# TianyiFranklinWang/MIRROR

Hardware: AMD Instinct MI355X
Metric: SSL samples/sec (slide+RNA pairs) (higher is better)
Workload: dtype bf16; 1 GPU; BASELINE c2: B=16/GPU x [4096 patch tokens x 1024-d] + [2048 genes], D=512, RNA depth 6 / 8 heads, train mode, local-batch InfoNCE; precision_policy=bf16, per_gpu_batch=16, global_batch=16, parallelism=dp1, grad_bucket_dtype=f32, step_launch=hip_graph

## Files before the change

### mirror_amd/csrc/resconv_mfma.hip

```cpp
#include <cstdlib>
#include "gemm_kernel.h"

namespace {

constexpr int RM_P = 72;
constexpr int RM_T = 128;
constexpr int RM_HALO = 16;
constexpr int RM_TAPS = 33;
constexpr int RM_DH = 64;
constexpr int RM_SP = 68;

typedef __attribute__((address_space(3))) s16x4 lds_s16x4;
typedef short s16x8 __attribute__((ext_vector_type(8)));
#define MFMA(a, b, c) __builtin_amdgcn_mfma_f32_32x32x16_bf16((a), (b), (c), 0, 0, 0)

__device__ __forceinline__ bf16x8 rm_frag_tr(const bf16_t* img, int col0, int kb, int lane) {
    const int g16 = lane >> 4, i = lane & 15, q = i >> 2, p = i & 3;
    const bf16_t* a0 = img + (kb + 4 * (g16 >> 1) + q) * RM_P + col0 + 16 * (g16 & 1) + 4 * p;
    s16x4 lo = __builtin_amdgcn_ds_read_tr16_b64_v4i16((lds_s16x4*)a0);
    s16x4 hi = __builtin_amdgcn_ds_read_tr16_b64_v4i16((lds_s16x4*)(a0 + 8 * RM_P));
    s16x8 v = __builtin_shufflevector(lo, hi, 0, 1, 2, 3, 4, 5, 6, 7);
    return __builtin_bit_cast(bf16x8, v);
}

__global__ __launch_bounds__(256) void resconv_mfma_kernel(const bf16_t* __restrict__ v, long ldv, long v_bs, const float* __restrict__ w,
                                                           bf16_t* out, long ldo, long o_bs, int n_p, int transpose, int accumulate) {
    static_assert(64 * RM_SP * 4 <= (RM_T + 2 * RM_HALO) * RM_P * 2, "half of the f32 output image must fit the v tile");
    __shared__ __attribute__((aligned(16))) bf16_t img[(RM_T + 2 * RM_HALO) * RM_P];
    const int tid = threadIdx.x, lane = tid & 63, wave = tid >> 6, hl = lane >> 5, r = lane & 31;
    const int t0 = blockIdx.x * RM_T, h = blockIdx.y, b = blockIdx.z;
    const bf16_t* vb = v + (long)b * v_bs + h * RM_DH;
#pragma unroll
    for (int i = 0; i < (RM_T + 2 * RM_HALO) * 8 / 256; i++) {
        const int cid = tid + i * 256, q = cid >> 3, c = cid & 7;
        const int t = t0 - RM_HALO + q;
        u32x4 val = {0u, 0u, 0u, 0u};
        if (t >= 0 && t < n_p) val = *reinterpret_cast<const u32x4*>(vb + (long)t * ldv + c * 8);
        *reinterpret_cast<u32x4*>(img + q * RM_P + c * 8) = val;
    }
    bf16_t* ob = out + (long)b * o_bs + h * RM_DH;
    u32x4 old[2][64 * 8 / 256];
    if (accumulate == 2) {
#pragma unroll
        for (int half = 0; half < 2; half++)
#pragma unroll
            for (int i = 0; i < 64 * 8 / 256; i++) {
                const int cid = tid + i * 256, q = cid >> 3, c = cid & 7;
                const int t = t0 + 64 * half + q;
                old[half][i] = (u32x4){0u, 0u, 0u, 0u};
                if (t < n_p) old[half][i] = *reinterpret_cast<const u32x4*>(ob + (long)t * ldo + 8 * c);
            }
    }
    const float* wh = w + h * RM_TAPS;
    bf16x8 wf[4];
#pragma unroll
    for (int ks = 0; ks < 4; ks++)
#pragma unroll
        for (int e = 0; e < 8; e++) {
            const int k = 16 * ks + (e < 4 ? 4 * hl + e : 8 + 4 * hl + (e - 4));
            const int j = k - r;
            const float x = (j >= 0 && j < RM_TAPS) ? wh[transpose ? RM_TAPS - 1 - j : j] : 0.f;
            wf[ks][e] = (__bf16)x;
        }
    __syncthreads();
    f32x16 acc[2];
#pragma unroll
    for (int nb = 0; nb < 2; nb++) {
#pragma unroll
        for (int e = 0; e < 16; e++) acc[nb][e] = 0.f;
#pragma unroll
        for (int ks = 0; ks < 4; ks++) acc[nb] = MFMA(rm_frag_tr(img, 32 * nb, 32 * wave + 16 * ks, lane), wf[ks], acc[nb]);
    }
    float* stage = reinterpret_cast<float*>(img);
    __syncthreads();
#pragma unroll
    for (int half = 0; half < 2; half++) {
        if ((wave >> 1) == half) {
            float* srow = stage + (32 * (wave & 1) + r) * RM_SP + 4 * hl;
#pragma unroll
            for (int nb = 0; nb < 2; nb++)
#pragma unroll
                for (int g = 0; g < 4; g++) {
                    f4_t x = {acc[nb][4 * g], acc[nb][4 * g + 1], acc[nb][4 * g + 2], acc[nb][4 * g + 3]};
                    *reinterpret_cast<f4_t*>(srow + 32 * nb + 8 * g) = x;
                }
        }
        __syncthreads();
#pragma unroll
        for (int i = 0; i < 64 * 8 / 256; i++) {
            const int cid = tid + i * 256, q = cid >> 3, c = cid & 7;
            const int t = t0 + 64 * half + q;
            if (t >= n_p) continue;
            const float* sp = stage + q * RM_SP + 8 * c;
            f4_t lo = *reinterpret_cast<const f4_t*>(sp), hi = *reinterpret_cast<const f4_t*>(sp + 4);
            bf16_t* p = ob + (long)t * ldo + 8 * c;
            if (accumulate) {
                const u32x4 od = accumulate == 2 ? old[half][i] : *reinterpret_cast<const u32x4*>(p);
                lo[0] += __uint_as_float(od[0] << 16); lo[1] += __uint_as_float(od[0] & 0xffff0000u);
                lo[2] += __uint_as_float(od[1] << 16); lo[3] += __uint_as_float(od[1] & 0xffff0000u);
                hi[0] += __uint_as_float(od[2] << 16); hi[1] += __uint_as_float(od[2] & 0xffff0000u);
                hi[2] += __uint_as_float(od[3] << 16); hi[3] += __uint_as_float(od[3] & 0xffff0000u);
            }
            u32x4 o;
            o[0] = pack_bf2(lo[0], lo[1]);
            o[1] = pack_bf2(lo[2], lo[3]);
            o[2] = pack_bf2(hi[0], hi[1]);
            o[3] = pack_bf2(hi[2], hi[3]);
            __builtin_nontemporal_store(o, reinterpret_cast<u32x4*>(p));
        }
        if (half == 0) __syncthreads();
    }
}

__global__ __launch_bounds__(256) void resconv_wgrad_mfma_kernel(const bf16_t* __restrict__ v, long ldv, long v_bs,
                                                                 const bf16_t* __restrict__ dout, long ldo, long o_bs,
                                                                 float* __restrict__ dw, int n_p) {
    __shared__ float gsum[64];
    __shared__ float s_S[4 * 32 * 65];
    const int tid = threadIdx.x, lane = tid & 63, wave = tid >> 6, hl = lane >> 5, r = lane & 31;
    const int h = blockIdx.y, b = blockIdx.z;
    if (tid < 64) gsum[tid] = 0.f;
    const bf16_t* vb = v + (long)b * v_bs + h * RM_DH + 8 * hl;
    const bf16_t* gb = dout + (long)b * o_bs + h * RM_DH + 8 * hl;
    f32x16 acc[2];
#pragma unroll
    for (int kb = 0; kb < 2; kb++)
#pragma unroll
        for (int e = 0; e < 16; e++) acc[kb][e] = 0.f;
    const int nblk = (n_p + 31) / 32;
    auto fetch = [&](int tb, bf16x8 (&af)[4], bf16x8 (&bf)[2][4]) {
        const int t = 32 * tb + r;
        const bool tok = t < n_p;
#pragma unroll
        for (int ks = 0; ks < 4; ks++) {
            u32x4 a = {0u, 0u, 0u, 0u};
            if (tok) a = *reinterpret_cast<const u32x4*>(gb + (long)t * ldo + 16 * ks);
            af[ks] = __builtin_bit_cast(bf16x8, a);
        }
#pragma unroll
        for (int kb = 0; kb < 2; kb++) {
            const int q = 32 * tb - RM_HALO + 32 * kb + r;
            const bool qok = q >= 0 && q < n_p;
#pragma unroll
            for (int ks = 0; ks < 4; ks++) {
                u32x4 x = {0u, 0u, 0u, 0u};
                if (qok) x = *reinterpret_cast<const u32x4*>(vb + (long)q * ldv + 16 * ks);
                bf[kb][ks] = __builtin_bit_cast(bf16x8, x);
            }
        }
    };
    auto mac = [&](const bf16x8 (&af)[4], const bf16x8 (&bf)[2][4]) {
#pragma unroll
        for (int kb = 0; kb < 2; kb++)
#pragma unroll
            for (int ks = 0; ks < 4; ks++) acc[kb] = MFMA(af[ks], bf[kb][ks], acc[kb]);
    };
    const int stride = 4 * gridDim.x;
    int tb = blockIdx.x * 4 + wave;
    bf16x8 a0[4], b0[2][4], a1[4], b1[2][4];
    if (tb < nblk) fetch(tb, a0, b0);
    while (tb < nblk) {
        if (tb + stride < nblk) fetch(tb + stride, a1, b1);
        mac(a0, b0);
        tb += stride;
        if (tb >= nblk) break;
        if (tb + stride < nblk) fetch(tb + stride, a0, b0);
        mac(a1, b1);
        tb += stride;
    }
    __syncthreads();
    float* S = s_S + wave * (32 * 65);
#pragma unroll
    for (int kb = 0; kb < 2; kb++)
#pragma unroll
        for (int e = 0; e < 16; e++) {
            const int i = 8 * (e >> 2) + 4 * hl + (e & 3);
            S[i * 65 + 32 * kb + r] = acc[kb][e];
        }
    __syncthreads();
    if (lane < RM_TAPS) {
        float t = 0.f;
#pragma unroll
        for (int i = 0; i < 32; i++) t += S[i * 65 + lane + i];
        atomicAdd(&gsum[lane], t);
    }
    __syncthreads();
    if (tid < RM_TAPS) atomicAdd(dw + h * RM_TAPS + tid, gsum[tid]);
}

__global__ __launch_bounds__(256, 3) void resconv_bwd_kernel(const bf16_t* __restrict__ dout, long ldo, long o_bs, const bf16_t* __restrict__ v,
                                                          long ldv, long v_bs, const float* __restrict__ w, bf16_t* dv, long lddv, long dv_bs,
                                                          float* __restrict__ part, int n_p) {
    static_assert(64 * RM_SP * 4 <= (RM_T + 2 * RM_HALO) * RM_P * 2, "half of the f32 output image must fit the dout tile");
    __shared__ __attribute__((aligned(16))) bf16_t img[(RM_T + 2 * RM_HALO) * RM_P];
    __shared__ float s_part[4][RM_TAPS + 1];
    const int tid = threadIdx.x, lane = tid & 63, wave = tid >> 6, hl = lane >> 5, r = lane & 31;
    const int t0 = blockIdx.x * RM_T, h = blockIdx.y, b = blockIdx.z;
    const bf16_t* gb = dout + (long)b * o_bs + h * RM_DH;
#pragma unroll
    for (int i = 0; i < (RM_T + 2 * RM_HALO) * 8 / 256; i++) {
        const int cid = tid + i * 256, q = cid >> 3, c = cid & 7;
        const int t = t0 - RM_HALO + q;
        u32x4 val = {0u, 0u, 0u, 0u};
        if (t >= 0 && t < n_p) val = *reinterpret_cast<const u32x4*>(gb + (long)t * ldo + c * 8);
        *reinterpret_cast<u32x4*>(img + q * RM_P + c * 8) = val;
    }
    bf16_t* ob = dv + (long)b * dv_bs + h * RM_DH;
    u32x4 old[2][64 * 8 / 256];
#pragma unroll
    for (int half = 0; half < 2; half++)
#pragma unroll
        for (int i = 0; i < 64 * 8 / 256; i++) {
            const int cid = tid + i * 256, q = cid >> 3, c = cid & 7;
            const int t = t0 + 64 * half + q;
            old[half][i] = (u32x4){0u, 0u, 0u, 0u};
            if (t < n_p) old[half][i] = *reinterpret_cast<const u32x4*>(ob + (long)t * lddv + 8 * c);
        }
    const bf16_t* vb = v + (long)b * v_bs + h * RM_DH + 8 * hl;
    bf16x8 bfv[2][4];
#pragma unroll
    for (int kb = 0; kb < 2; kb++) {
        const int q = t0 + 32 * wave - RM_HALO + 32 * kb + r;
        const bool qok = q >= 0 && q < n_p;
#pragma unroll
        for (int ks = 0; ks < 4; ks++) {
            u32x4 x = {0u, 0u, 0u, 0u};
            if (qok) x = *reinterpret_cast<const u32x4*>(vb + (long)q * ldv + 16 * ks);
            bfv[kb][ks] = __builtin_bit_cast(bf16x8, x);
        }
    }
    const float* wh = w + h * RM_TAPS;
    bf16x8 wf[4];
#pragma unroll
    for (int ks = 0; ks < 4; ks++)
#pragma unroll
        for (int e = 0; e < 8; e++) {
            const int k = 16 * ks + (e < 4 ? 4 * hl + e : 8 + 4 * hl + (e - 4));
            const int j = k - r;
            const float x = wh[RM_TAPS - 1 - min(max(j, 0), RM_TAPS - 1)];
            wf[ks][e] = (__bf16)((j >= 0 && j < RM_TAPS) ? x : 0.f);
        }
    __syncthreads();
    f32x16 acc[2], S[2];
#pragma unroll
    for (int nb = 0; nb < 2; nb++) {
#pragma unroll
        for (int e = 0; e < 16; e++) acc[nb][e] = S[nb][e] = 0.f;
#pragma unroll
        for (int ks = 0; ks < 4; ks++) acc[nb] = MFMA(rm_frag_tr(img, 32 * nb, 32 * wave + 16 * ks, lane), wf[ks], acc[nb]);
    }
#pragma unroll
    for (int ks = 0; ks < 4; ks++) {
        const bf16x8 af = *reinterpret_cast<const bf16x8*>(img + (RM_HALO + 32 * wave + r) * RM_P + 16 * ks + 8 * hl);
#pragma unroll
        for (int kb = 0; kb < 2; kb++) S[kb] = MFMA(af, bfv[kb][ks], S[kb]);
    }
    float tsum = 0.f, t32 = 0.f;
#pragma unroll
    for (int e = 0; e < 16; e++) {
        const int i = 8 * (e >> 2) + 4 * hl + (e & 3);
        const float val = (r >= i) ? S[0][e] : S[1][e];
        t32 += (r == i) ? S[1][e] : 0.f;
        const int src = 32 * hl + ((r + i) & 31);
        tsum += __builtin_bit_cast(float, __builtin_amdgcn_ds_bpermute(src << 2, __builtin_bit_cast(int, val)));
    }
    tsum += __shfl_xor(tsum, 32, 64);
#pragma unroll
    for (int o = 32; o > 0; o >>= 1) t32 += __shfl_xor(t32, o, 64);
    if (lane < 32) s_part[wave][lane] = tsum;
    if (lane == 0) s_part[wave][32] = t32;
    float* stage = reinterpret_cast<float*>(img);
    __syncthreads();
    if (tid < RM_TAPS)
        part[(((long)b * gridDim.y + h) * gridDim.x + blockIdx.x) * RM_TAPS + tid] = s_part[0][tid] + s_part[1][tid] + s_part[2][tid] + s_part[3][tid];
#pragma unroll
    for (int half = 0; half < 2; half++) {
        if ((wave >> 1) == half) {
            float* srow = stage + (32 * (wave & 1) + r) * RM_SP + 4 * hl;
#pragma unroll
            for (int nb = 0; nb < 2; nb++)
#pragma unroll
                for (int g = 0; g < 4; g++) {
                    f4_t x = {acc[nb][4 * g], acc[nb][4 * g + 1], acc[nb][4 * g + 2], acc[nb][4 * g + 3]};
                    *reinterpret_cast<f4_t*>(srow + 32 * nb + 8 * g) = x;
                }
        }
        __syncthreads();
#pragma unroll
        for (int i = 0; i < 64 * 8 / 256; i++) {
            const int cid = tid + i * 256, q = cid >> 3, c = cid & 7;
            const int t = t0 + 64 * half + q;
            if (t >= n_p) continue;
            const float* sp = stage + q * RM_SP + 8 * c;
            f4_t lo = *reinterpret_cast<const f4_t*>(sp), hi = *reinterpret_cast<const f4_t*>(sp + 4);
            const u32x4 od = old[half][i];
            lo[0] += __uint_as_float(od[0] << 16); lo[1] += __uint_as_float(od[0] & 0xffff0000u);
            lo[2] += __uint_as_float(od[1] << 16); lo[3] += __uint_as_float(od[1] & 0xffff0000u);
            hi[0] += __uint_as_float(od[2] << 16); hi[1] += __uint_as_float(od[2] & 0xffff0000u);
            hi[2] += __uint_as_float(od[3] << 16); hi[3] += __uint_as_float(od[3] & 0xffff0000u);
            u32x4 o;
            o[0] = pack_bf2(lo[0], lo[1]);
            o[1] = pack_bf2(lo[2], lo[3]);
            o[2] = pack_bf2(hi[0], hi[1]);
            o[3] = pack_bf2(hi[2], hi[3]);
            *reinterpret_cast<u32x4*>(ob + (long)t * lddv + 8 * c) = o;
        }
        if (half == 0) __syncthreads();
    }
}

__global__ __launch_bounds__(256) void resconv_bwd_fold_kernel(const float* __restrict__ part, float* __restrict__ dw, int tiles) {
    __shared__ float red[4][64];
    const int h = blockIdx.x, b = blockIdx.y, j = threadIdx.x & 63, q = threadIdx.x >> 6;
    const float* pb = part + ((long)b * gridDim.x + h) * tiles * RM_TAPS;
    float s = 0.f;
    if (j < RM_TAPS) {
        int t = q;
        for (; t + 12 < tiles; t += 16) {
            const float a0 = pb[(long)t * RM_TAPS + j], a1 = pb[(long)(t + 4) * RM_TAPS + j], a2 = pb[(long)(t + 8) * RM_TAPS + j],
                        a3 = pb[(long)(t + 12) * RM_TAPS + j];
            s += (a0 + a1) + (a2 + a3);
        }
        for (; t < tiles; t += 4) s += pb[(long)t * RM_TAPS + j];
    }
    red[q][j] = s;
    __syncthreads();
    if (q == 0 && j < RM_TAPS) atomicAdd(dw + h * RM_TAPS + j, red[0][j] + red[1][j] + red[2][j] + red[3][j]);
}

}

long resconv_bwd_part_floats(int B, int n_p, int heads, int dh, int taps) {
    if (dh != RM_DH || taps != RM_TAPS || B <= 0 || n_p <= 0) return 0;
    return (long)B * heads * mh_cdiv(n_p, RM_T) * RM_TAPS;
}

bool resconv_bwd_try_mfma(const void* dout, long ldo, long o_bs, const void* v, long ldv, long v_bs, const float* w, void* dv, long lddv,
                          long dv_bs, float* dw, float* part, long part_floats, int B, int n_p, int heads, int dh, int taps, int dt,
                          hipStream_t s) {
    if (dt != MH_BF16 || dh != RM_DH || taps != RM_TAPS) return false;
    if (ldv % 8 || v_bs % 8 || ldo % 8 || o_bs % 8 || lddv % 8 || dv_bs % 8 || ((uintptr_t)v & 15) || ((uintptr_t)dout & 15) || ((uintptr_t)dv & 15))
        return false;
    if (!part || part_floats < resconv_bwd_part_floats(B, n_p, heads, dh, taps)) return false;
    const int tiles = mh_cdiv(n_p, RM_T);
    hipLaunchKernelGGL(resconv_bwd_kernel, dim3(tiles, heads, B), dim3(256), 0, s, (const bf16_t*)dout, ldo, o_bs, (const bf16_t*)v, ldv, v_bs,
                       w, (bf16_t*)dv, lddv, dv_bs, part, n_p);
    hipLaunchKernelGGL(resconv_bwd_fold_kernel, dim3(heads, B), dim3(256), 0, s, (const float*)part, dw, tiles);
    return true;
}

bool resconv_try_mfma(const void* v, long ldv, long v_bs, const float* w, void* out, long ldo, long o_bs, int B, int n_p, int heads,
                      int dh, int taps, int transpose, int accumulate, int dt_v, int dt_o, hipStream_t s) {
    if (dt_v != MH_BF16 || dt_o != MH_BF16 || dh != RM_DH || taps != RM_TAPS) return false;
    if (ldv % 8 || v_bs % 8 || ldo % 8 || o_bs % 8 || ((uintptr_t)v & 15) || ((uintptr_t)out & 15)) return false;
    dim3 grid(mh_cdiv(n_p, RM_T), heads, B);
    constexpr bool early = true;
    hipLaunchKernelGGL(resconv_mfma_kernel, grid, dim3(256), 0, s, (const bf16_t*)v, ldv, v_bs, w, (bf16_t*)out, ldo, o_bs, n_p,
                       transpose, accumulate ? (early ? 2 : 1) : 0);
    return true;
}

bool resconv_wgrad_try_mfma(const void* v, long ldv, long v_bs, const void* dout, long ldo, long o_bs, float* dw, int B, int n_p,
                            int heads, int dh, int taps, int dt_v, int dt_o, hipStream_t s) {
    if (dt_v != MH_BF16 || dt_o != MH_BF16 || dh != RM_DH || taps != RM_TAPS) return false;
    if (ldv % 8 || v_bs % 8 || ldo % 8 || o_bs % 8 || ((uintptr_t)v & 15) || ((uintptr_t)dout & 15)) return false;
    const int nblk = mh_cdiv(n_p, 32);
    int splits = 1;
    constexpr int target = 256;
    while (splits * 2 * heads * B <= target && splits * 2 * 4 <= nblk) splits *= 2;
    dim3 grid(splits, heads, B);
    hipLaunchKernelGGL(resconv_wgrad_mfma_kernel, grid, dim3(256), 0, s, (const bf16_t*)v, ldv, v_bs, (const bf16_t*)dout, ldo, o_bs,
                       dw, n_p);
    return true;
}
```

Measured before the change: 2239 samples/s.

## Make residual-conv backward kernel persistent over tile ranges with prefetch and halo reuse

```diff
diff --git a/mirror_amd/csrc/resconv_mfma.hip b/mirror_amd/csrc/resconv_mfma.hip
--- a/mirror_amd/csrc/resconv_mfma.hip
+++ b/mirror_amd/csrc/resconv_mfma.hip
@@ -1,4 +1,5 @@
 #include <cstdlib>
+#include <type_traits>
 #include "gemm_kernel.h"
 
 namespace {
@@ -188,124 +189,174 @@
     if (tid < RM_TAPS) atomicAdd(dw + h * RM_TAPS + tid, gsum[tid]);
 }
 
-__global__ __launch_bounds__(256, 3) void resconv_bwd_kernel(const bf16_t* __restrict__ dout, long ldo, long o_bs, const bf16_t* __restrict__ v,
+__global__ __launch_bounds__(256, 2) void resconv_bwd_kernel(const bf16_t* __restrict__ dout, long ldo, long o_bs, const bf16_t* __restrict__ v,
                                                           long ldv, long v_bs, const float* __restrict__ w, bf16_t* dv, long lddv, long dv_bs,
-                                                          float* __restrict__ part, int n_p) {
-    static_assert(64 * RM_SP * 4 <= (RM_T + 2 * RM_HALO) * RM_P * 2, "half of the f32 output image must fit the dout tile");
+                                                          float* __restrict__ part, int n_p, int tiles) {
     __shared__ __attribute__((aligned(16))) bf16_t img[(RM_T + 2 * RM_HALO) * RM_P];
+    __shared__ __attribute__((aligned(16))) float stage[64 * RM_SP];
+    __shared__ __attribute__((aligned(16))) bf16x8 s_wf[4][64];
     __shared__ float s_part[4][RM_TAPS + 1];
     const int tid = threadIdx.x, lane = tid & 63, wave = tid >> 6, hl = lane >> 5, r = lane & 31;
-    const int t0 = blockIdx.x * RM_T, h = blockIdx.y, b = blockIdx.z;
+    const int h = blockIdx.y, b = blockIdx.z;
+    const int tile_lo = (int)((long)blockIdx.x * tiles / gridDim.x), tile_hi = (int)((long)(blockIdx.x + 1) * tiles / gridDim.x);
     const bf16_t* gb = dout + (long)b * o_bs + h * RM_DH;
-#pragma unroll
-    for (int i = 0; i < (RM_T + 2 * RM_HALO) * 8 / 256; i++) {
-        const int cid = tid + i * 256, q = cid >> 3, c = cid & 7;
-        const int t = t0 - RM_HALO + q;
-        u32x4 val = {0u, 0u, 0u, 0u};
-        if (t >= 0 && t < n_p) val = *reinterpret_cast<const u32x4*>(gb + (long)t * ldo + c * 8);
-        *reinterpret_cast<u32x4*>(img + q * RM_P + c * 8) = val;
-    }
     bf16_t* ob = dv + (long)b * dv_bs + h * RM_DH;
-    u32x4 old[2][64 * 8 / 256];
-#pragma unroll
-    for (int half = 0; half < 2; half++)
-#pragma unroll
-        for (int i = 0; i < 64 * 8 / 256; i++) {
-            const int cid = tid + i * 256, q = cid >> 3, c = cid & 7;
-            const int t = t0 + 64 * half + q;
-            old[half][i] = (u32x4){0u, 0u, 0u, 0u};
-            if (t < n_p) old[half][i] = *reinterpret_cast<const u32x4*>(ob + (long)t * lddv + 8 * c);
-        }
     const bf16_t* vb = v + (long)b * v_bs + h * RM_DH + 8 * hl;
-    bf16x8 bfv[2][4];
-#pragma unroll
-    for (int kb = 0; kb < 2; kb++) {
-        const int q = t0 + 32 * wave - RM_HALO + 32 * kb + r;
-        const bool qok = q >= 0 && q < n_p;
-#pragma unroll
-        for (int ks = 0; ks < 4; ks++) {
-            u32x4 x = {0u, 0u, 0u, 0u};
-            if (qok) x = *reinterpret_cast<const u32x4*>(vb + (long)q * ldv + 16 * ks);
-            bfv[kb][ks] = __builtin_bit_cast(bf16x8, x);
-        }
-    }
-    const float* wh = w + h * RM_TAPS;
-    bf16x8 wf[4];
-#pragma unroll
-    for (int ks = 0; ks < 4; ks++)
+    const int rq = tid >> 3, rc = 8 * (tid & 7);
+    auto fetch_rows = [&](int t0, u32x4 (&nd)[4], u32x4 (&no)[4]) {
+#pragma unroll
+        for (int i = 0; i < 4; i++) nd[i] = *reinterpret_cast<const u32x4*>(gb + (long)min(t0 + RM_HALO + rq + 32 * i, n_p - 1) * ldo + rc);
+#pragma unroll
+        for (int i = 0; i < 4; i++) no[i] = *reinterpret_cast<const u32x4*>(ob + (long)min(t0 + rq + 32 * i, n_p - 1) * lddv + rc);
+    };
+    auto fetch_v = [&](int t0, bf16x8 (&nb)[2][4]) {
+#pragma unroll
+        for (int kb = 0; kb < 2; kb++) {
+            const int q = t0 + 32 * wave - RM_HALO + 32 * kb + r;
+            const bf16_t* p = vb + (long)min(max(q, 0), n_p - 1) * ldv;
+#pragma unroll
+            for (int ks = 0; ks < 4; ks++) nb[kb][ks] = __builtin_bit_cast(bf16x8, *reinterpret_cast<const u32x4*>(p + 16 * ks));
+        }
+    };
+    auto refill = [&](int t0, const u32x4 (&nd)[4]) {
+        const u32x4 keep = *reinterpret_cast<const u32x4*>(img + (RM_T + rq) * RM_P + rc);
+        *reinterpret_cast<u32x4*>(img + rq * RM_P + rc) = keep;
+#pragma unroll
+        for (int i = 0; i < 4; i++) {
+            const int q = rq + 32 * i;
+            const u32x4 zero = {0u, 0u, 0u, 0u};
+            *reinterpret_cast<u32x4*>(img + (2 * RM_HALO + q) * RM_P + rc) = (t0 + RM_HALO + q < n_p) ? nd[i] : zero;
+        }
+    };
+    u32x4 oldA[4], oldB[4];
+    bf16x8 bfvA[2][4], bfvB[2][4];
+    {
+        const int t0 = tile_lo * RM_T;
+        u32x4 nd[4];
+        const int tl = t0 - RM_HALO + rq;
+        const u32x4 lead = *reinterpret_cast<const u32x4*>(gb + (long)min(max(tl, 0), n_p - 1) * ldo + rc);
+        fetch_rows(t0, nd, oldA);
+        fetch_v(t0, bfvA);
+        const u32x4 zero = {0u, 0u, 0u, 0u};
+        *reinterpret_cast<u32x4*>(img + rq * RM_P + rc) = (tl >= 0 && tl < n_p) ? lead : zero;
+#pragma unroll
+        for (int i = 0; i < 4; i++) {
+            const int q = rq + 32 * i;
+            *reinterpret_cast<u32x4*>(img + (2 * RM_HALO + q) * RM_P + rc) = (t0 + RM_HALO + q < n_p) ? nd[i] : zero;
+        }
+    }
+    {
+        const float* wh = w + h * RM_TAPS;
+        const int ks = wave;
+        bf16x8 wf;
 #pragma unroll
         for (int e = 0; e < 8; e++) {
             const int k = 16 * ks + (e < 4 ? 4 * hl + e : 8 + 4 * hl + (e - 4));
             const int j = k - r;
             const float x = wh[RM_TAPS - 1 - min(max(j, 0), RM_TAPS - 1)];
-            wf[ks][e] = (__bf16)((j >= 0 && j < RM_TAPS) ? x : 0.f);
-        }
-    __syncthreads();
-    f32x16 acc[2], S[2];
-#pragma unroll
-    for (int nb = 0; nb < 2; nb++) {
-#pragma unroll
-        for (int e = 0; e < 16; e++) acc[nb][e] = S[nb][e] = 0.f;
-#pragma unroll
-        for (int ks = 0; ks < 4; ks++) acc[nb] = MFMA(rm_frag_tr(img, 32 * nb, 32 * wave + 16 * ks, lane), wf[ks], acc[nb]);
-    }
-#pragma unroll
-    for (int ks = 0; ks < 4; ks++) {
-        const bf16x8 af = *reinterpret_cast<const bf16x8*>(img + (RM_HALO + 32 * wave + r) * RM_P + 16 * ks + 8 * hl);
-#pragma unroll
-        for (int kb = 0; kb < 2; kb++) S[kb] = MFMA(af, bfv[kb][ks], S[kb]);
-    }
-    float tsum = 0.f, t32 = 0.f;
-#pragma unroll
-    for (int e = 0; e < 16; e++) {
-        const int i = 8 * (e >> 2) + 4 * hl + (e & 3);
-        const float val = (r >= i) ? S[0][e] : S[1][e];
-        t32 += (r == i) ? S[1][e] : 0.f;
-        const int src = 32 * hl + ((r + i) & 31);
-        tsum += __builtin_bit_cast(float, __builtin_amdgcn_ds_bpermute(src << 2, __builtin_bit_cast(int, val)));
-    }
-    tsum += __shfl_xor(tsum, 32, 64);
-#pragma unroll
-    for (int o = 32; o > 0; o >>= 1) t32 += __shfl_xor(t32, o, 64);
-    if (lane < 32) s_part[wave][lane] = tsum;
-    if (lane == 0) s_part[wave][32] = t32;
-    float* stage = reinterpret_cast<float*>(img);
-    __syncthreads();
-    if (tid < RM_TAPS)
-        part[(((long)b * gridDim.y + h) * gridDim.x + blockIdx.x) * RM_TAPS + tid] = s_part[0][tid] + s_part[1][tid] + s_part[2][tid] + s_part[3][tid];
-#pragma unroll
-    for (int half = 0; half < 2; half++) {
-        if ((wave >> 1) == half) {
-            float* srow = stage + (32 * (wave & 1) + r) * RM_SP + 4 * hl;
-#pragma unroll
-            for (int nb = 0; nb < 2; nb++)
-#pragma unroll
-                for (int g = 0; g < 4; g++) {
-                    f4_t x = {acc[nb][4 * g], acc[nb][4 * g + 1], acc[nb][4 * g + 2], acc[nb][4 * g + 3]};
-                    *reinterpret_cast<f4_t*>(srow + 32 * nb + 8 * g) = x;
-                }
+            wf[e] = (__bf16)((j >= 0 && j < RM_TAPS) ? x : 0.f);
+        }
+        s_wf[ks][lane] = wf;
+    }
+    __syncthreads();
+    auto step = [&](int tile, auto more_c, u32x4 (&old)[4], bf16x8 (&bfv)[2][4], u32x4 (&no)[4], bf16x8 (&nb)[2][4]) __attribute__((always_inline)) {
+        constexpr bool more = decltype(more_c)::value;
+        const int t0 = tile * RM_T;
+        u32x4 nd[4];
+        if constexpr (more) fetch_rows(t0 + RM_T, nd, no);
+        f32x16 acc[2], S[2];
+#pragma unroll
+        for (int kb = 0; kb < 2; kb++) {
+            const int q = t0 + 32 * wave - RM_HALO + 32 * kb + r;
+            const bool qok = q >= 0 && q < n_p;
+            const bf16x8 zero = __builtin_bit_cast(bf16x8, (u32x4){0u, 0u, 0u, 0u});
+#pragma unroll
+            for (int ks = 0; ks < 4; ks++) bfv[kb][ks] = qok ? bfv[kb][ks] : zero;
+#pragma unroll
+            for (int e = 0; e < 16; e++) acc[kb][e] = S[kb][e] = 0.f;
+        }
+#pragma unroll
+        for (int ks = 0; ks < 4; ks++) {
+            const bf16x8 af = *reinterpret_cast<const bf16x8*>(img + (RM_HALO + 32 * wave + r) * RM_P + 16 * ks + 8 * hl);
+#pragma unroll
+            for (int kb = 0; kb < 2; kb++) S[kb] = MFMA(af, bfv[kb][ks], S[kb]);
+        }
+        float tsum = 0.f, t32 = 0.f;
+#pragma unroll
+        for (int e = 0; e < 16; e++) {
+            const int i = 8 * (e >> 2) + 4 * hl + (e & 3);
+            const float val = (r >= i) ? S[0][e] : S[1][e];
+            t32 += (r == i) ? S[1][e] : 0.f;
+            const int src = 32 * hl + ((r + i) & 31);
+            tsum += __builtin_bit_cast(float, __builtin_amdgcn_ds_bpermute(src << 2, __builtin_bit_cast(int, val)));
+        }
+        tsum += __shfl_xor(tsum, 32, 64);
+#pragma unroll
+        for (int o = 32; o > 0; o >>= 1) t32 += __shfl_xor(t32, o, 64);
+        if (lane < 32) s_part[wave][lane] = tsum;
+        if (lane == 0) s_part[wave][32] = t32;
+        __builtin_amdgcn_sched_barrier(0);
+        if constexpr (more) fetch_v(t0 + RM_T, nb);
+#pragma unroll
+        for (int ks = 0; ks < 4; ks++) {
+            const bf16x8 wf = s_wf[ks][lane];
+#pragma unroll
+            for (int nc = 0; nc < 2; nc++) acc[nc] = MFMA(rm_frag_tr(img, 32 * nc, 32 * wave + 16 * ks, lane), wf, acc[nc]);
         }
         __syncthreads();
-#pragma unroll
-        for (int i = 0; i < 64 * 8 / 256; i++) {
-            const int cid = tid + i * 256, q = cid >> 3, c = cid & 7;
-            const int t = t0 + 64 * half + q;
-            if (t >= n_p) continue;
-            const float* sp = stage + q * RM_SP + 8 * c;
-            f4_t lo = *reinterpret_cast<const f4_t*>(sp), hi = *reinterpret_cast<const f4_t*>(sp + 4);
-            const u32x4 od = old[half][i];
-            lo[0] += __uint_as_float(od[0] << 16); lo[1] += __uint_as_float(od[0] & 0xffff0000u);
-            lo[2] += __uint_as_float(od[1] << 16); lo[3] += __uint_as_float(od[1] & 0xffff0000u);
-            hi[0] += __uint_as_float(od[2] << 16); hi[1] += __uint_as_float(od[2] & 0xffff0000u);
-            hi[2] += __uint_as_float(od[3] << 16); hi[3] += __uint_as_float(od[3] & 0xffff0000u);
-            u32x4 o;
-            o[0] = pack_bf2(lo[0], lo[1]);
-            o[1] = pack_bf2(lo[2], lo[3]);
-            o[2] = pack_bf2(hi[0], hi[1]);
-            o[3] = pack_bf2(hi[2], hi[3]);
-            *reinterpret_cast<u32x4*>(ob + (long)t * lddv + 8 * c) = o;
-        }
-        if (half == 0) __syncthreads();
+        if (tid < RM_TAPS)
+            part[(((long)b * gridDim.y + h) * tiles + tile) * RM_TAPS + tid] = s_part[0][tid] + s_part[1][tid] + s_part[2][tid] + s_part[3][tid];
+#pragma unroll
+        for (int half = 0; half < 2; half++) {
+            if ((wave >> 1) == half) {
+                float* srow = stage + (32 * (wave & 1) + r) * RM_SP + 4 * hl;
+#pragma unroll
+                for (int nc = 0; nc < 2; nc++)
+#pragma unroll
+                    for (int g = 0; g < 4; g++) {
+                        f4_t x = {acc[nc][4 * g], acc[nc][4 * g + 1], acc[nc][4 * g + 2], acc[nc][4 * g + 3]};
+                        *reinterpret_cast<f4_t*>(srow + 32 * nc + 8 * g) = x;
+                    }
+            }
+            __syncthreads();
+#pragma unroll
+            for (int i = 0; i < 2; i++) {
+                const int q = rq + 32 * i;
+                const int t = t0 + 64 * half + q;
+                if (t >= n_p) continue;
+                const float* sp = stage + q * RM_SP + rc;
+                f4_t lo = *reinterpret_cast<const f4_t*>(sp), hi = *reinterpret_cast<const f4_t*>(sp + 4);
+                const u32x4 od = old[2 * half + i];
+                lo[0] += __uint_as_float(od[0] << 16); lo[1] += __uint_as_float(od[0] & 0xffff0000u);
+                lo[2] += __uint_as_float(od[1] << 16); lo[3] += __uint_as_float(od[1] & 0xffff0000u);
+                hi[0] += __uint_as_float(od[2] << 16); hi[1] += __uint_as_float(od[2] & 0xffff0000u);
+                hi[2] += __uint_as_float(od[3] << 16); hi[3] += __uint_as_float(od[3] & 0xffff0000u);
+                u32x4 o;
+                o[0] = pack_bf2(lo[0], lo[1]);
+                o[1] = pack_bf2(lo[2], lo[3]);
+                o[2] = pack_bf2(hi[0], hi[1]);
+                o[3] = pack_bf2(hi[2], hi[3]);
+                *reinterpret_cast<u32x4*>(ob + (long)t * lddv + rc) = o;
+            }
+            if (half == 0) __syncthreads();
+        }
+        if constexpr (more) {
+            refill(t0 + RM_T, nd);
+            __syncthreads();
+        }
+    };
+    const std::true_type yes;
+    const std::false_type no_more;
+    int tile = tile_lo;
+    for (; tile + 2 < tile_hi; tile += 2) {
+        step(tile, yes, oldA, bfvA, oldB, bfvB);
+        step(tile + 1, yes, oldB, bfvB, oldA, bfvA);
+    }
+    if (tile + 2 == tile_hi) {
+        step(tile, yes, oldA, bfvA, oldB, bfvB);
+        step(tile + 1, no_more, oldB, bfvB, oldA, bfvA);
+    } else {
+        step(tile, no_more, oldA, bfvA, oldB, bfvB);
     }
 }
 
@@ -343,8 +394,14 @@
         return false;
     if (!part || part_floats < resconv_bwd_part_floats(B, n_p, heads, dh, taps)) return false;
     const int tiles = mh_cdiv(n_p, RM_T);
-    hipLaunchKernelGGL(resconv_bwd_kernel, dim3(tiles, heads, B), dim3(256), 0, s, (const bf16_t*)dout, ldo, o_bs, (const bf16_t*)v, ldv, v_bs,
-                       w, (bf16_t*)dv, lddv, dv_bs, part, n_p);
+    int ranges = mh_cdiv(tiles, 2);
+    if ((long)ranges * heads * B < 256) ranges = tiles;
+    if (const char* e = getenv("MH_RESCONV_BWD_RANGES")) {
+        const int forced = atoi(e);
+        if (forced >= 1) ranges = std::min(forced, tiles);
+    }
+    hipLaunchKernelGGL(resconv_bwd_kernel, dim3(ranges, heads, B), dim3(256), 0, s, (const bf16_t*)dout, ldo, o_bs, (const bf16_t*)v, ldv, v_bs,
+                       w, (bf16_t*)dv, lddv, dv_bs, part, n_p, tiles);
     hipLaunchKernelGGL(resconv_bwd_fold_kernel, dim3(heads, B), dim3(256), 0, s, (const float*)part, dw, tiles);
     return true;
 }
```

Result: no change. 2244 samples/s (median of 6 runs) (+0.2%).
